# soedinglab/MMseqs2

Measured on AMD Instinct MI355X. Metric: sw_gcells_per_s, higher is better.
Workload: dtype int16

## Files before the change

### mmseqs2_amd/csrc/mmgpu_internal.h

```cpp
#ifndef MMGPU_INTERNAL_H
#define MMGPU_INTERNAL_H

#include <hip/hip_runtime.h>
#include <stdint.h>
#include <cstdlib>
#include <cstring>

#include <algorithm>
#include <array>
#include <string>
#include <map>
#include <mutex>
#include <chrono>
#include <memory>
#include <vector>
#include <thread>
#include <atomic>

#include "../../include/mmgpu.h"
#include "nucl_core.h"
#include "block_plan.h"

namespace mmgpu {

struct DeviceDb {
    uint8_t *res = nullptr;
    uint32_t *off4 = nullptr;
    uint32_t *len = nullptr;
    uint32_t n = 0;
    uint32_t max_len = 0;
    uint64_t total_residues = 0;
    int alphabet = 0;
    size_t res_bytes = 0;
};

struct TargetView {
    const uint8_t *res = nullptr;
    const uint32_t *off4 = nullptr;
    const uint32_t *len = nullptr;
    uint32_t n = 0;
    uint32_t max_len = 0;
    const uint32_t *h_len = nullptr;
};

struct SwMaskGatherArgs {
    const uint8_t *src_res;
    const uint32_t *src_off4, *src_len;
    const uint32_t *src_id;
    uint8_t *dst_res;
    const uint32_t *dst_off4;
    const uint32_t *span_off;
    const mmgpu_sw_span *spans;
    uint32_t span_base;
    uint32_t mask_letter;
    uint32_t n_pairs;
};
hipError_t launch_sw_mask_gather(const SwMaskGatherArgs &A, hipStream_t stream);

struct SwJob {
    uint32_t query;
    uint32_t hit_begin;
    uint32_t hit_end;
    uint32_t shape;
};

struct SwLaunch {
    const SwJob *jobs;
    uint32_t n_jobs;
    const uint8_t *q_res;
    const int8_t *q_cb;
    const uint32_t *q_off;
    const int32_t *q_bias;
    const int32_t *q_minstart;
    const int8_t *q_prof;
    const uint32_t *q_prof_off;
    const uint8_t *t_res;
    const uint32_t *t_off4;
    const uint32_t *t_len;
    const uint32_t *hit_target;
    const uint32_t *hit_out;
    mmgpu_sw_hit *out;
    const int8_t *mat;
    int alphabet;
    int gap_open, gap_extend;
    uint2 *scratch;
    uint32_t scratch_cols;
    uint32_t *scratch_busy;
    uint32_t scratch_slots;
    uint32_t resident_lds = 0;
    const uint32_t *q_hit_count;
    uint32_t hit_stride;
    int rev_mode = 0;
    int rev_only = 0;
    const uint8_t *rev_force = nullptr;
    int half_wide = 1;
};

constexpr int SW_PF_MAX_LIST = 16384;
constexpr int SW_FROM_PF_STAT_SLOTS = 64;

struct SwFromPfArgs {
    const mmgpu_pf_hit *pf_hits;
    uint32_t pf_stride;
    const uint32_t *hit_count;
    uint32_t stride;
    const uint32_t *q_off;
    const uint32_t *t_len;
    uint32_t *hit_target, *hit_out;
    unsigned long long *cells, *pairs;
    uint32_t *count_copy;
    uint32_t *slot_target;
};

constexpr int SW_REV_JOB_MAX = 1024;
hipError_t launch_sw_rev_multi(const SwLaunch &L, size_t lds_bytes, hipStream_t stream);
hipError_t launch_sw_from_pf(const SwFromPfArgs &A, uint32_t nq, hipStream_t stream);
uint32_t sw_multi_resident_blocks(size_t lds_bytes, bool both_passes, int compute_units);

#ifndef MMGPU_SW_MAX_R
#define MMGPU_SW_MAX_R 28
#endif
constexpr int SW_MAX_R = MMGPU_SW_MAX_R;
static_assert(SW_MAX_R >= 16 && SW_MAX_R <= 32, "multi-tile bodies exist for 8..32 rows per lane: a query cut into tiles gets at least SW_MAX_R / 2");
#ifndef MMGPU_SW_MIN_WAVES
#define MMGPU_SW_MIN_WAVES 2
#endif
constexpr int SW_MIN_WAVES = MMGPU_SW_MIN_WAVES;
#ifndef MMGPU_SW_GROUPS
#define MMGPU_SW_GROUPS 4
#endif
constexpr int SW_GROUPS = MMGPU_SW_GROUPS;
static_assert(SW_GROUPS == 3 || SW_GROUPS == 4, "three or four kernel groups");
constexpr int SW_GROUP0_MAX_R = 12;
constexpr int SW_GROUP1_MAX_R = 24;
__host__ __device__ constexpr int sw_group_of(bool multi, int R) {
    return multi ? SW_GROUPS - 1 : (R <= SW_GROUP0_MAX_R ? 0 : (R <= SW_GROUP1_MAX_R ? 1 : 2));
}
int sw_shape_group(uint32_t shape);
hipError_t launch_sw(const SwLaunch &L, int group, size_t lds_bytes, bool both_passes, hipStream_t stream);
#ifndef MMGPU_SW_HALF
#define MMGPU_SW_HALF 1
#endif
bool launch_sw_half(const SwLaunch &L, int group, size_t lds_bytes, bool both_passes, hipStream_t stream);
void warm_sw_half();

constexpr int SW_LDS_HEADER = SW_REV_JOB_MAX * 2 + 64;
__host__ __device__ constexpr int lane_stride_bytes(int R) {
    int slots = (R * 2 + 15) / 16;
    if ((slots & 1) == 0) slots += 1;
    return slots * 16;
}
__host__ __device__ constexpr uint32_t sw_profile_bytes(int R, int alphabet, int lanes = 16) {
    return (uint32_t)(alphabet + 1) * (uint32_t)lanes * (uint32_t)lane_stride_bytes(R);
}
#ifndef MMGPU_SW_RESIDENT_LDS
#define MMGPU_SW_RESIDENT_LDS 65536
#endif
constexpr uint32_t SW_RESIDENT_LDS = MMGPU_SW_RESIDENT_LDS;
static_assert(SW_RESIDENT_LDS <= 65536u, "a workgroup asks for at most 64 KB of dynamic LDS");
__host__ __device__ constexpr uint32_t sw_tiles(uint32_t qlen, int R) { return (qlen + 16u * (uint32_t)R - 1u) / (16u * (uint32_t)R); }
__host__ __device__ constexpr bool sw_multi_resident(uint32_t n_tiles, int R, int alphabet, uint32_t budget) {
    return (unsigned long long)n_tiles * sw_profile_bytes(R, alphabet) + (unsigned long long)SW_LDS_HEADER <= (unsigned long long)budget;
}
static_assert(sw_multi_resident(2, 28, 21, 65536) && sw_multi_resident(3, 24, 21, 65536) && !sw_multi_resident(3, 25, 21, 65536) &&
              !sw_multi_resident(4, 22, 21, 65536) && !sw_multi_resident(2, 8, 21, 0), "residency rule");

constexpr uint32_t SW_SHAPE_MULTI = 32, SW_SHAPE_WIDE = 64;
constexpr int SW_WIDE_MIN_R = (16 * SW_MAX_R + 1 + 31) / 32;
static_assert(sw_profile_bytes(SW_MAX_R, 21, 32) == 2 * sw_profile_bytes(SW_MAX_R, 21) &&
              sw_profile_bytes(SW_MAX_R, 21, 32) + SW_LDS_HEADER <= 65536u, "a wide tile fits a workgroup's 64 KB");
static_assert((lane_stride_bytes(SW_MAX_R) / 16) % 2 == 1 && (lane_stride_bytes(SW_WIDE_MIN_R) / 16) % 2 == 1, "odd number of 16-byte slots");
bool sw_wide_enabled();
bool sw_half_wide();

constexpr int SCAN_CLASSES = 5;
constexpr int SCAN_MULTI = SCAN_CLASSES - 1;
constexpr int SCAN_MAX_R = 32;
constexpr int SCAN_ROUND = 32;
constexpr int SCAN_JOB_TARGETS = 16 * SCAN_ROUND;
__host__ __device__ constexpr int scan_class_rows(int cls) { return cls == 0 ? 8 : cls == 1 ? 16 : cls == 2 ? 24 : 32; }
__host__ __device__ constexpr uint32_t scan_cols(uint32_t len, int R) { return (len + (uint32_t)R - 1u) / (uint32_t)R * (uint32_t)R; }
__host__ __device__ constexpr uint32_t scan_park_row_words(uint32_t longest) { return 2u * ((scan_cols(longest, SCAN_MAX_R) + 1u + 15u) & ~15u); }

constexpr uint64_t SCAN_NO_PROFILE = ~0ull;

struct ScanJob {
    uint32_t query;
    uint32_t begin, end;
    uint32_t pad;
};

struct ScanLaunch {
    const ScanJob *jobs;
    uint32_t n_jobs;
    const uint8_t *q_res;
    const int8_t *q_cb;
    const uint32_t *q_off;
    const int32_t *q_cap;
    const int8_t *q_prof;
    const uint64_t *q_prof_off;
    const uint32_t *q_prof_letters;
    const uint8_t *t_res;
    const uint32_t *t_off4, *t_len;
    const uint32_t *order;
    uint32_t n_targets;
    const int8_t *mat;
    int alphabet;
    uint8_t *scores;
    uint32_t *park;
    const uint64_t *park_off;
};
hipError_t launch_scan(const ScanLaunch &L, int cls, uint32_t grid, hipStream_t stream);

struct ScanSelectArgs {
    const uint8_t *scores;
    const uint32_t *t_len;
    uint32_t n_targets;
    const uint32_t *q_ident;
    const uint32_t *q_win;
    int32_t min_score;
    uint32_t max_hits;
    mmgpu_pf_hit *hits;
    uint32_t stride;
    uint32_t *counts;
};
hipError_t launch_scan_select(const ScanSelectArgs &A, uint32_t nq, hipStream_t stream);
void warm_scan();

constexpr uint64_t GSCAN_PAIR_BUDGET = 1ull << 24;

struct SwDenseLists {
    const uint32_t *begin, *count;
    const uint32_t *order;
    const uint64_t *len_prefix;
    uint32_t *d_hit_target, *d_hit_out;
    mmgpu_sw_hit *d_out;
};

struct GscanPlanArgs {
    const uint32_t *order;
    const uint32_t *q_begin, *q_count;
    const uint32_t *q_slot;
    uint32_t q_first, n_queries;
    uint32_t *hit_target, *hit_out;
};
hipError_t launch_gscan_plan(const GscanPlanArgs &A, hipStream_t stream);

struct GscanIdentArgs {
    const uint8_t *q_res;
    const int8_t *q_cb;
    const uint32_t *q_off;
    const int8_t *q_prof;
    const uint32_t *q_prof_off;
    const uint32_t *q_ident;
    const uint8_t *t_res;
    const uint32_t *t_off4;
    const int8_t *mat;
    int alphabet;
    int32_t *ident_score;
};
hipError_t launch_gscan_identity(const GscanIdentArgs &A, uint32_t nq, hipStream_t stream);

struct GscanSelectArgs {
    const mmgpu_sw_hit *out;
    const uint32_t *order;
    const uint32_t *q_begin, *q_count, *q_slot;
    const uint32_t *q_ident;
    const int32_t *ident_score;
    const int32_t *q_min_ev;
    const uint32_t *t_len;
    const uint32_t *q_win;
    int32_t *scores;
    uint32_t n_targets;
    uint32_t q_first;
    int32_t min_score;
    uint32_t max_hits;
    mmgpu_pf_hit *hits;
    uint32_t stride;
    uint32_t *counts;
};
hipError_t launch_gscan_select(const GscanSelectArgs &A, uint32_t n_queries, hipStream_t stream);
void warm_gscan();

constexpr int RESCORE_GROUP = 16;
constexpr int RESCORE_STEP = 4;
constexpr int RESCORE_THREADS = 256;
constexpr int RESCORE_SLACK = 16;

struct RescoreArgs {
    const uint8_t *q_res;
    const uint32_t *q_off4, *q_len;
    const uint8_t *t_res;
    const uint32_t *t_off4, *t_len;
    const int8_t *mat;
    int alphabet;
    const uint32_t *hit_query;
    const mmgpu_rescore_pair *pairs;
// ... 813 lines not shown
```

### mmseqs2_amd/csrc/sw_body.h

```cpp
#pragma once
#include "mmgpu_internal.h"
#include "pf_device.h"

namespace mmgpu {

namespace {

constexpr int GROUP = 16;
constexpr int WAVES = 4;
constexpr int GROUPS_PER_WAVE = 64 / GROUP;
constexpr int HITS_PER_WAVE = 2 * GROUPS_PER_WAVE;
constexpr unsigned NEG2 = 0x80008000u;

typedef short s16x2 __attribute__((ext_vector_type(2)));
typedef unsigned short u16x2 __attribute__((ext_vector_type(2)));

__device__ __forceinline__ unsigned pk_add_sat(unsigned a, unsigned b) {
    return __builtin_bit_cast(unsigned, __builtin_elementwise_add_sat(__builtin_bit_cast(s16x2, a),
                                                                      __builtin_bit_cast(s16x2, b)));
}
__device__ __forceinline__ unsigned pk_max_s(unsigned a, unsigned b) {
    return __builtin_bit_cast(unsigned, __builtin_elementwise_max(__builtin_bit_cast(s16x2, a),
                                                                  __builtin_bit_cast(s16x2, b)));
}
__device__ __forceinline__ unsigned pk_max_u(unsigned a, unsigned b) {
    return __builtin_bit_cast(unsigned, __builtin_elementwise_max(__builtin_bit_cast(u16x2, a),
                                                                  __builtin_bit_cast(u16x2, b)));
}
__device__ __forceinline__ unsigned pk_sub_sat_u(unsigned a, unsigned b) {
    return __builtin_bit_cast(unsigned, __builtin_elementwise_sub_sat(__builtin_bit_cast(u16x2, a),
                                                                      __builtin_bit_cast(u16x2, b)));
}
__device__ __forceinline__ unsigned bfi(unsigned mask, unsigned a, unsigned b) {
    return (a & mask) | (b & ~mask);
}

constexpr int SW_HALF_LIMIT = 2048 - 256;
constexpr int SW_HALF_MAX_GAP = 2048;
constexpr int SW_HALF_MARK = -1;
typedef _Float16 h16x2 __attribute__((ext_vector_type(2)));
__device__ __forceinline__ h16x2 as_h(unsigned a) { return __builtin_bit_cast(h16x2, a); }
__device__ __forceinline__ unsigned as_u(h16x2 a) { return __builtin_bit_cast(unsigned, a); }
__device__ __forceinline__ unsigned h_add(unsigned a, unsigned b) { return as_u(as_h(a) + as_h(b)); }
__device__ __forceinline__ unsigned h_sub(unsigned a, unsigned b) { return as_u(as_h(a) - as_h(b)); }
__device__ __forceinline__ unsigned h_max(unsigned a, unsigned b) {
    return as_u(__builtin_elementwise_maximum(as_h(a), as_h(b)));
}
__device__ __forceinline__ unsigned h_max3(unsigned a, unsigned b, unsigned c) {
    return as_u(__builtin_elementwise_maximum(__builtin_elementwise_maximum(as_h(a), as_h(b)), as_h(c)));
}
__device__ __forceinline__ unsigned short h_bits(int v) { return __builtin_bit_cast(unsigned short, (_Float16)v); }
__device__ __forceinline__ int h_value(unsigned bits) { return (int)(float)__builtin_bit_cast(_Float16, (unsigned short)bits); }
template <int W>
__device__ __forceinline__ unsigned across_rows(unsigned x, unsigned v) {
    static_assert(W == 16 || W == 32, "groups of one or two DPP rows");
    if constexpr (W == 32) x = __builtin_amdgcn_update_dpp(x, v, 0x138 , 0xA, 0x1, false);
    return x;
}
template <int W = GROUP>
__device__ __forceinline__ unsigned from_lane_above(unsigned head, unsigned v) {
    return across_rows<W>(__builtin_amdgcn_update_dpp(head, v, 0x111 , 0xF, 0xF, false), v);
}
template <int W = GROUP>
__device__ __forceinline__ unsigned from_lane_above_or_zero(unsigned v) {
    return across_rows<W>(__builtin_amdgcn_update_dpp(0u, v, 0x111 , 0xF, 0xF, true), v);
}

#ifndef MMGPU_SW_PREFETCH
#define MMGPU_SW_PREFETCH 1
#endif
#define SW_KEEP_IN_ROW(x) asm volatile("" : "+v"(x))

template <int R, int W = GROUP>
struct Tile {
    static constexpr int ROWS = W * R;
    static constexpr int LANE_STRIDE = lane_stride_bytes(R);
    static constexpr int ROW_STRIDE = W * LANE_STRIDE;
};
static_assert(GROUP == 16, "sw_profile_bytes' default and sw_tiles (mmgpu_internal.h) assume 16-lane groups for all but the wide shapes");

template <int R, bool REV, bool HALF = false, int W = GROUP>
__device__ __forceinline__ void build_profile(unsigned char *lds, const uint8_t *q, const int8_t *cb, int qlen,
                                              int tile_base, const int8_t *mat, int alphabet, const int8_t *prof) {
    using T = Tile<R, W>;
    const int total = (alphabet + 1) * T::ROWS;
    for (int idx = threadIdx.x; idx < total; idx += blockDim.x) {
        const int letter = idx / T::ROWS;
        const int row = idx - letter * T::ROWS;
        const int rg = tile_base + row;
        short v = (short)-32768;
        if (letter < alphabet && rg < qlen) {
            const int qi = REV ? (qlen - 1 - rg) : rg;
            v = prof ? (short)prof[letter * qlen + qi] : (short)((int)mat[letter * alphabet + q[qi]] + (int)cb[qi]);
        }
        const int lane = row / R, r = row - lane * R;
        if constexpr (HALF) v = (short)h_bits(v);
        *reinterpret_cast<short *>(lds + letter * T::ROW_STRIDE + lane * T::LANE_STRIDE + r * 2) = v;
    }
}

__device__ __forceinline__ bool sw_rev_wanted(const SwLaunch &L, uint32_t slot, int min_start) {
    const mmgpu_sw_hit &f = L.out[slot];
    const int s = f.score;
    if (L.rev_mode == 2) return s > 0 && L.rev_force[slot] != 0;
    return s > 0 && s >= min_start && !(L.rev_mode == 1 && f.word != 0);
}

constexpr int SW_REV_JOB_HITS = 1024;
static_assert(SW_REV_JOB_HITS == SW_REV_JOB_MAX, "host and kernel disagree on the reverse job size");
struct SwLds {
    uint16_t live[SW_REV_JOB_HITS];
    uint32_t live_wave[WAVES];
    uint32_t next_chunk;
    uint32_t half_flag;
    uint32_t unused[10];
    __device__ unsigned char *profiles() { return reinterpret_cast<unsigned char *>(this + 1); }
};
constexpr int SW_HALF_FLAG_AT = offsetof(SwLds, half_flag);
static_assert(SW_LDS_HEADER == SW_REV_JOB_HITS * 2 + 64 && sizeof(SwLds) == SW_LDS_HEADER && SW_HALF_FLAG_AT == SW_REV_JOB_HITS * 2 + 20 &&
              offsetof(SwLds, next_chunk) == SW_REV_JOB_HITS * 2 + 16, "the header holds the live hits and the scheduling words");
__device__ __forceinline__ SwLds &sw_lds() {
    extern __shared__ __attribute__((aligned(16))) unsigned char lds_all[];
    return *reinterpret_cast<SwLds *>(lds_all);
}
__device__ __forceinline__ uint32_t sw_half_any_marked() { return sw_lds().half_flag; }

struct SwQuery {
    const uint8_t *q;
    const int8_t *cb;
    int qlen, qbias;
    const int8_t *prof;
};
__device__ __forceinline__ SwQuery sw_query(const SwLaunch &L, uint32_t query) {
    const uint32_t qbeg = L.q_off[query];
    SwQuery Q;
    Q.qlen = (int)(L.q_off[query + 1] - qbeg);
    Q.q = L.q_res + qbeg;
    Q.cb = L.q_cb + qbeg;
    Q.qbias = L.q_bias[query];
    Q.prof = nullptr;
    if (L.q_prof_off) {
        const uint32_t po = L.q_prof_off[query];
        if (po != 0xFFFFFFFFu) Q.prof = L.q_prof + po;
    }
    return Q;
}

struct SwProfiles {
    unsigned char *lds;
    int n_tiles;
    uint32_t tile_bytes;
    bool resident;
    bool dynamic;
};
template <int R, bool MULTI>
__device__ __forceinline__ SwProfiles sw_profiles(const SwLaunch &L, int qlen) {
    SwProfiles P;
    P.lds = sw_lds().profiles();
    P.n_tiles = MULTI ? (int)sw_tiles((uint32_t)qlen, R) : 1;
    P.tile_bytes = sw_profile_bytes(R, L.alphabet);
    P.resident = MULTI && sw_multi_resident((uint32_t)P.n_tiles, R, L.alphabet, L.resident_lds);
    P.dynamic = !MULTI || P.resident;
    return P;
}
enum SwBuildAt { SW_AT_JOB_START, SW_AT_PACKED, SW_AT_TILE };
template <SwBuildAt AT, int R, bool REV, bool HALF, bool PACKED, int W>
__device__ __forceinline__ void sw_build_profiles(const SwLaunch &L, const SwQuery &Q, const SwProfiles &P, int tile = 0) {
    using T = Tile<R, W>;
    if (AT == SW_AT_TILE) {
        if (!P.dynamic) {
            __syncthreads();
            build_profile<R, REV, HALF, W>(P.lds, Q.q, Q.cb, Q.qlen, tile * T::ROWS, L.mat, L.alphabet, Q.prof);
            __syncthreads();
        }
    } else if ((AT == SW_AT_PACKED) == PACKED && P.dynamic) {
        for (int t = 0; t < P.n_tiles; ++t)
            build_profile<R, REV, HALF, W>(P.lds + (uint32_t)t * P.tile_bytes, Q.q, Q.cb, Q.qlen, t * T::ROWS, L.mat, L.alphabet, Q.prof);
        __syncthreads();
    }
}

template <bool REV, bool MARKED>
__device__ __forceinline__ uint32_t sw_pack_live(const SwLaunch &L, const SwJob &job, SwLds &H, uint32_t n_hits) {
    const int lane = threadIdx.x & 63;
    const int wave = __builtin_amdgcn_readfirstlane(threadIdx.x >> 6);
    const int min_start = REV ? L.q_minstart[job.query] : 0;
    uint32_t total = 0;
    for (uint32_t base = 0; base < n_hits; base += WAVES * 64) {
        const uint32_t idx = base + threadIdx.x;
        bool pass = false;
        if (idx < n_hits) {
            const uint32_t slot = L.hit_out[job.hit_begin + idx];
            pass = MARKED ? L.out[slot].score == SW_HALF_MARK : sw_rev_wanted(L, slot, min_start);
        }
        const unsigned long long bal = __ballot(pass);
        if (lane == 0) H.live_wave[wave] = (uint32_t)__popcll(bal);
        __syncthreads();
        uint32_t before = 0, round_total = 0;
#pragma unroll
        for (int w = 0; w < WAVES; ++w) {
            const uint32_t c = H.live_wave[w];
            before += w < wave ? c : 0u;
            round_total += c;
        }
        if (pass) H.live[total + before + (uint32_t)__popcll(bal & ((1ull << lane) - 1ull))] = (uint16_t)idx;
        total += round_total;
        __syncthreads();
    }
    return total;
}

template <int W>
__device__ __forceinline__ uint32_t sw_claim_chunk(SwLds &H, bool dynamic, uint32_t it) {
    constexpr int HITS_PER_WAVE = 2 * 64 / W;
    const int lane = threadIdx.x & 63;
    const int wave = __builtin_amdgcn_readfirstlane(threadIdx.x >> 6);
    uint32_t chunk = it * WAVES + wave;
    if (dynamic) {
        if (lane == 0) chunk = atomicAdd(&H.next_chunk, 1u);
        chunk = __builtin_amdgcn_readfirstlane(chunk);
    }
    return chunk * HITS_PER_WAVE;
}

template <bool REV, bool HALF>
__device__ __forceinline__ void sw_write_result(const SwLaunch &L, const SwQuery &Q, unsigned long long key, uint32_t h, int end, int cols) {
    const bool marked = HALF && (unsigned)(key >> 32) > (unsigned)h_bits(SW_HALF_LIMIT);
    const int score = HALF ? (marked ? SW_HALF_MARK : h_value((unsigned)(key >> 32))) : (int)(key >> 32);
    const int col = 0xFFFF - (int)((key >> 16) & 0xFFFFu);
    const int row = 0xFFFF - (int)(key & 0xFFFFu);
    mmgpu_sw_hit *o = L.out + L.hit_out[h];
    if (!REV) {
        mmgpu_sw_hit res;
        res.score = score;
        res.q_end = score ? row : 0;
        res.t_end = score ? col : -1;
        res.q_start = -1;
        res.t_start = -1;
        res.word = (score + Q.qbias >= 255) ? 1 : 0;
        *o = res;
        if (marked) sw_lds().half_flag = 1;
    } else {
        if (cols > 0) {
            o->t_start = (score == o->score) ? end - col : -2;
            o->q_start = (score == o->score) ? Q.qlen - 1 - row : -2;
        }
    }
}

template <int R, bool MULTI, bool REV, bool PF, bool HALF = false, bool MARKED = false, int W = GROUP>
__device__ __forceinline__ void sw_body(const SwLaunch &L, const SwJob job) {
    static_assert(!(HALF || MARKED) || (!MULTI && !REV && !(HALF && MARKED)), "f16 and its int16 re-run: single-tile forward scans");
    static_assert(W == GROUP || (W == 2 * GROUP && !MULTI), "the boundary row of a multi-tile body rotates inside one DPP row");
    constexpr bool PACKED = REV || MARKED;
    constexpr int HITS_PER_WAVE = 2 * 64 / W;
    using T = Tile<R, W>;
    SwLds &H = sw_lds();
    if (MULTI) __builtin_amdgcn_s_setprio(3);
    const int lane = threadIdx.x & 63;
    const int wave = __builtin_amdgcn_readfirstlane(threadIdx.x >> 6);
    const int g = lane & (W - 1);
    const int grp = lane / W;
    const SwQuery Q = sw_query(L, job.query);
    const SwProfiles prof = sw_profiles<R, MULTI>(L, Q.qlen);
    const unsigned go2 = (HALF ? (unsigned)h_bits(L.gap_open) : (unsigned)L.gap_open) * 0x10001u;
    const unsigned ge2 = (HALF ? (unsigned)h_bits(L.gap_extend) : (unsigned)L.gap_extend) * 0x10001u;
    const unsigned pad_letter = (unsigned)L.alphabet;

    if (threadIdx.x == 0) H.next_chunk = 0;
    if (HALF && threadIdx.x == 0) H.half_flag = 0;
    sw_build_profiles<SW_AT_JOB_START, R, REV, HALF, PACKED, W>(L, Q, prof);
    uint32_t n_hits = job.hit_end - job.hit_begin;
    if (PACKED) {
        n_hits = sw_pack_live<REV, MARKED>(L, job, H, n_hits);
        if (n_hits == 0) return;
    }
    sw_build_profiles<SW_AT_PACKED, R, REV, HALF, PACKED, W>(L, Q, prof);
    const uint32_t n_iter = (n_hits + WAVES * HITS_PER_WAVE - 1) / (WAVES * HITS_PER_WAVE);

    for (uint32_t it = 0; prof.dynamic || it < n_iter; ++it) {
        const uint32_t slot0 = sw_claim_chunk<W>(H, prof.dynamic, it);
        if (prof.dynamic && slot0 >= n_hits) break;

        const uint32_t sA = slot0 + grp * 2, sB = sA + 1;
        const bool vA = sA < n_hits, vB = sB < n_hits;
        const uint32_t hA = job.hit_begin + (PACKED ? (uint32_t)H.live[vA ? sA : 0] : sA);
        const uint32_t hB = job.hit_begin + (PACKED ? (uint32_t)H.live[vB ? sB : 0] : sB);
        const uint32_t tA = vA ? L.hit_target[hA] : 0u, tB = vB ? L.hit_target[hB] : 0u;
        const uint8_t *pA = L.t_res + (size_t)L.t_off4[tA] * 4;
        const uint8_t *pB = L.t_res + (size_t)L.t_off4[tB] * 4;
        int colsA = vA ? (int)L.t_len[tA] : 0, colsB = vB ? (int)L.t_len[tB] : 0;
        int r0A = 0, r0B = 0;
        int endA = 0, endB = 0;
        unsigned rev_target = 0xFFFFFFFFu;
        if (REV) {
            mmgpu_sw_hit fa, fb;
            fa.score = 0; fa.q_end = 0; fa.t_end = 0;
            fb = fa;
            if (vA) fa = L.out[L.hit_out[hA]];
            if (vB) fb = L.out[L.hit_out[hB]];
            colsA = vA ? fa.t_end + 1 : 0;
            colsB = vB ? fb.t_end + 1 : 0;
            endA = colsA > 0 ? fa.t_end : 0;
            endB = colsB > 0 ? fb.t_end : 0;
            r0A = colsA > 0 ? Q.qlen - 1 - fa.q_end : 0;
            r0B = colsB > 0 ? Q.qlen - 1 - fb.q_end : 0;
            rev_target = (colsA > 0 ? (unsigned)fa.score & 0xFFFFu : 0xFFFFu) | ((colsB > 0 ? (unsigned)fb.score & 0xFFFFu : 0xFFFFu) << 16);
        }
        int ncols = colsA > colsB ? colsA : colsB;
        ncols = max(ncols, __shfl_xor(ncols, 16));
        ncols = max(ncols, __shfl_xor(ncols, 32));
        ncols = __builtin_amdgcn_readfirstlane(ncols);
        const int nsteps = ncols + W - 1;
        int mincols = colsA < colsB ? colsA : colsB;
        mincols = min(mincols, __shfl_xor(mincols, 16));
        mincols = min(mincols, __shfl_xor(mincols, 32));
        mincols = __builtin_amdgcn_readfirstlane(mincols);

        unsigned long long bestA = 0, bestB = 0;

        uint2 *scr = nullptr;
        unsigned scr_grp = 0;
        if (MULTI) {
            scr = L.scratch + (size_t)((job.shape >> 8) * WAVES + wave) * GROUPS_PER_WAVE * 2 * L.scratch_cols;
            scr_grp = (unsigned)grp * 2u * L.scratch_cols;
        }

        for (int tile = 0; tile < prof.n_tiles; ++tile) {
            const int tile_base = tile * T::ROWS;
            sw_build_profiles<SW_AT_TILE, R, REV, HALF, PACKED, W>(L, Q, prof, tile);
            const unsigned char *const lds_tile = MULTI && prof.resident ? prof.lds + (uint32_t)tile * prof.tile_bytes : prof.lds;
            const uint2 *scr_in = MULTI ? scr + (size_t)((tile + 1) & 1) * L.scratch_cols : nullptr;
            uint2 *scr_out = MULTI ? scr + (size_t)(tile & 1) * L.scratch_cols : nullptr;
            const bool has_above = MULTI && tile > 0;
            const bool has_below = MULTI && tile + 1 < prof.n_tiles;

            unsigned Hp[R], E[R], aux[R];
#pragma unroll
            for (int r = 0; r < R; ++r) { Hp[r] = 0; E[r] = 0; aux[r] = 0; }
            if (REV) {
#pragma unroll
                for (int r = 0; r < R; ++r) {
                    const int rg = tile_base + g * R + r;
                    aux[r] = (rg >= r0A ? 0xFFFFu : 0u) | (rg >= r0B ? 0xFFFF0000u : 0u);
                }
            }
            unsigned vmax = 0, bestcol = 0xFFFFFFFFu;
            unsigned rev_rowA = 0, rev_rowB = 0;
            unsigned Hup_prev = 0;
            unsigned out_H = 0, out_F = 0;

            auto letters4 = [&](const uint8_t *p, int end, int k) -> unsigned {
                if (!REV) return reinterpret_cast<const unsigned *>(p)[k];
                int o = end - 3 - 4 * k;
                o = o < -3 ? -3 : o;
                unsigned w;
                __builtin_memcpy(&w, p + o, 4);
                return w;
            };
            unsigned wA = letters4(pA, endA, 0), wB = letters4(pB, endB, 0);
            unsigned wA_next = letters4(pA, endA, 1), wB_next = letters4(pB, endB, 1);
            uint2 bnd = make_uint2(0, 0), bnd_next = make_uint2(0, 0);
            auto boundary16 = [&](int m) -> uint2 {
                const int last = ncols - 1 < 0 ? 0 : ncols - 1;
                return scr_in[scr_grp + (unsigned)min(16 * m + g - (m > 0 ? 1 : 0), last)];
            };
            if (has_above) {
                bnd = boundary16(0);
                bnd_next = boundary16(1);
            }

            constexpr int ND = (R + 1) / 2;
            unsigned pav_next[PF ? ND : 1], pbv_next[PF ? ND : 1];
            auto load_rows = [&](unsigned letters, unsigned *pav, unsigned *pbv) {
                const unsigned a = letters & 0xFFu, b = (letters >> 8) & 0xFFu;
                const uint4 *rowA = reinterpret_cast<const uint4 *>(lds_tile + a * T::ROW_STRIDE + g * T::LANE_STRIDE);
                const uint4 *rowB = reinterpret_cast<const uint4 *>(lds_tile + b * T::ROW_STRIDE + g * T::LANE_STRIDE);
#pragma unroll
                for (int k = 0; k < ND / 4; ++k) {
                    const uint4 pa = rowA[k], pb = rowB[k];
                    pav[4 * k] = pa.x; pav[4 * k + 1] = pa.y; pav[4 * k + 2] = pa.z; pav[4 * k + 3] = pa.w;
                    pbv[4 * k] = pb.x; pbv[4 * k + 1] = pb.y; pbv[4 * k + 2] = pb.z; pbv[4 * k + 3] = pb.w;
                }
                if constexpr (ND % 4 >= 2) {
                    const uint2 pa = *reinterpret_cast<const uint2 *>(rowA + ND / 4);
                    const uint2 pb = *reinterpret_cast<const uint2 *>(rowB + ND / 4);
                    pav[(ND / 4) * 4] = pa.x; pav[(ND / 4) * 4 + 1] = pa.y;
                    pbv[(ND / 4) * 4] = pb.x; pbv[(ND / 4) * 4 + 1] = pb.y;
                }
                if constexpr (ND % 2 == 1) {
                    pav[ND - 1] = reinterpret_cast<const unsigned *>(rowA)[ND - 1];
                    pbv[ND - 1] = reinterpret_cast<const unsigned *>(rowB)[ND - 1];
                }
            };
            unsigned let = pad_letter * 0x101u;
            constexpr bool LETTER_BLOCKS = MULTI || REV || R >= 7;
            constexpr bool LETTER_QUEUE = !MULTI && R < 7;
            unsigned long long lq = 0;
            auto letter_block = [&](int k) {
                if (!LETTER_BLOCKS) return;
                unsigned a = wA, b = wB;
                if (4 * k + 4 > mincols) {
                    const unsigned pad4 = pad_letter * 0x01010101u;
                    const int na = min(max(colsA - 4 * k, 0), 4), nb = min(max(colsB - 4 * k, 0), 4);
                    const unsigned ma = REV ? ~(unsigned)(0xFFFFFFFFull >> (8 * na)) : (unsigned)((1ull << (8 * na)) - 1ull);
                    const unsigned mb = REV ? ~(unsigned)(0xFFFFFFFFull >> (8 * nb)) : (unsigned)((1ull << (8 * nb)) - 1ull);
                    a = bfi(ma, a, pad4);
                    b = bfi(mb, b, pad4);
                }
                const unsigned lo = __builtin_amdgcn_perm(b, a, REV ? 0x06020703u : 0x05010400u);
                const unsigned hi = __builtin_amdgcn_perm(b, a, REV ? 0x04000501u : 0x07030602u);
                lq = ((unsigned long long)hi << 32) | lo;
            };
            auto head_letters = [&](int c, int j) -> unsigned {
                if (LETTER_BLOCKS && LETTER_QUEUE) { const unsigned v = (unsigned)lq; lq >>= 16; return v; }
                if (LETTER_BLOCKS) return (unsigned)(lq >> (16 * j));
                const unsigned sh = (unsigned)(REV ? 3 - j : j) * 8u;
                const unsigned la0 = __builtin_amdgcn_ubfe(wA, sh, 8u);
                const unsigned lb0 = __builtin_amdgcn_ubfe(wB, sh, 8u);
                return (c < colsA ? la0 : pad_letter) | ((c < colsB ? lb0 : pad_letter) << 8);
            };
            letter_block(0);
            let = from_lane_above<W>(head_letters(0, 0), let);
            if (PF) load_rows(let, pav_next, pbv_next);

            for (int s0 = -1; s0 < nsteps; s0 += 4) {
            if (MULTI && s0 > 0 && ((s0 + 1) & 15) == 0) {
                bnd = bnd_next;
                if (has_above) bnd_next = boundary16(((s0 + 1) >> 4) + 1);
            }
            const int jn = min(4, nsteps - s0);
#pragma nounroll
            for (int j = s0 < 0 ? 1 : 0; j < jn; ++j) {
                const int s = s0 + j;
                if (has_below && s >= GROUP) {
                    if (g == GROUP - 1) (scr_out + (s - GROUP))[scr_grp] = make_uint2(out_H, out_F);
                }
                const unsigned Hup = MULTI ? from_lane_above<W>(bnd.x, out_H) : from_lane_above_or_zero<W>(out_H);
                unsigned f = MULTI ? from_lane_above<W>(bnd.y, out_F) : from_lane_above_or_zero<W>(out_F);
                if (MULTI) {
                    bnd.x = __builtin_amdgcn_update_dpp(bnd.x, bnd.x, 0x12F, 0xF, 0xF, false);
                    bnd.y = __builtin_amdgcn_update_dpp(bnd.y, bnd.y, 0x12F, 0xF, 0xF, false);
                }
                unsigned pav[ND], pbv[ND];
                if (PF) {
#pragma unroll
                    for (int k = 0; k < ND; ++k) { pav[k] = pav_next[k]; pbv[k] = pbv_next[k]; }
                } else {
                    load_rows(let, pav, pbv);
                }

                unsigned hd = Hup_prev;
                Hup_prev = Hup;
                unsigned cmax = 0;
                unsigned pre[R], es[R];
#pragma unroll
                for (int r = 0; r < R; ++r) {
                    unsigned P = __builtin_amdgcn_perm(pbv[r / 2], pav[r / 2], (r & 1) ? 0x07060302u : 0x05040100u);
                    if (REV) P = __builtin_amdgcn_bitop3_b32(aux[r], P, NEG2, 0xCA);
                    if constexpr (HALF) {
                        pre[r] = h_add(r == 0 ? hd : Hp[r - 1], P);
                        es[r] = h_sub(E[r], ge2);
                    } else {
                        pre[r] = pk_max_s(pk_add_sat(r == 0 ? hd : Hp[r - 1], P), E[r]);
                        es[r] = pk_sub_sat_u(E[r], ge2);
                    }
                }
                let = from_lane_above<W>(head_letters(s + 1, j), let);
                if (PF) load_rows(let, pav_next, pbv_next);
#pragma unroll
                for (int r = 0; r < R; ++r) {
                    unsigned h;
                    if constexpr (HALF) {
                        h = h_max3(pre[r], E[r], f);
                        const unsigned fs = h_sub(f, ge2);
                        const unsigned t = h_sub(h, go2);
                        cmax = r == 0 ? h : h_max(cmax, h);
                        f = h_max3(fs, t, 0u);
                        E[r] = h_max3(es[r], t, 0u);
                    } else {
                        h = pk_max_s(pre[r], f);
                        const unsigned fs = pk_sub_sat_u(f, ge2);
                        const unsigned t = pk_sub_sat_u(h, go2);
                        cmax = pk_max_u(cmax, h);
                        f = pk_max_u(fs, t);
                        E[r] = pk_max_u(es[r], t);
                    }
                    SW_KEEP_IN_ROW(E[r]);
                    Hp[r] = h;
                }
                out_H = Hp[R - 1];
                out_F = f;

                const int col = s - g;

                const unsigned nm = pk_max_u(vmax, cmax);
                if (nm != vmax) {
                    const unsigned diff = nm ^ vmax;
                    if (!REV) {
                        const unsigned mask = ((diff & 0xFFFFu) ? 0xFFFFu : 0u) | ((diff >> 16) ? 0xFFFF0000u : 0u);
                        bestcol = bfi(mask, ((unsigned)col & 0xFFFFu) * 0x10001u, bestcol);
#pragma unroll
                        for (int r = 0; r < R; ++r) aux[r] = bfi(mask, Hp[r], aux[r]);
                    } else {
                        const unsigned x = nm ^ rev_target;
                        const bool hitA = (diff & 0xFFFFu) && !(x & 0xFFFFu), hitB = (diff >> 16) && !(x >> 16);
                        if (hitA | hitB) {
                            asm volatile("" ::: "memory");
                            unsigned ra = 0, rb = 0;
#pragma unroll
                            for (int r = R - 1; r >= 0; --r) {
                                if ((Hp[r] & 0xFFFFu) == (rev_target & 0xFFFFu)) ra = (unsigned)r;
                                if ((Hp[r] >> 16) == (rev_target >> 16)) rb = (unsigned)r;
                            }
                            if (hitA) { bestcol = (bestcol & 0xFFFF0000u) | ((unsigned)col & 0xFFFFu); rev_rowA = ra; }
                            if (hitB) { bestcol = (bestcol & 0xFFFFu) | ((unsigned)col << 16); rev_rowB = rb; }
                        }
                    }
                    vmax = nm;
                }
            }
            {
                wA = wA_next; wB = wB_next;
                const int k = ((s0 + 1) >> 2) + 2;
                wA_next = letters4(pA, endA, k); wB_next = letters4(pB, endB, k);
                letter_block(k - 1);
            }
            }
            if (has_below && ncols > 0 && g == GROUP - 1) (scr_out + (ncols - 1))[scr_grp] = make_uint2(out_H, out_F);

            unsigned rowA_first = rev_rowA, rowB_first = rev_rowB;
            unsigned sA = vmax & 0xFFFFu, sB = vmax >> 16;
            if (!REV) {
#pragma unroll
                for (int r = R - 1; r >= 0; --r) {
                    if ((aux[r] & 0xFFFFu) == sA) rowA_first = (unsigned)r;
                    if ((aux[r] >> 16) == sB) rowB_first = (unsigned)r;
                }
            } else {
                sA = sA == (rev_target & 0xFFFFu) ? sA : 0u;
                sB = sB == (rev_target >> 16) ? sB : 0u;
            }
            const unsigned rgA = (unsigned)(tile_base + g * R) + rowA_first;
            const unsigned rgB = (unsigned)(tile_base + g * R) + rowB_first;
            unsigned long long keyA = sA ? ((unsigned long long)sA << 32) | ((0xFFFFu - (bestcol & 0xFFFFu)) << 16) | (0xFFFFu - rgA) : 0ull;
            unsigned long long keyB = sB ? ((unsigned long long)sB << 32) | ((0xFFFFu - (bestcol >> 16)) << 16) | (0xFFFFu - rgB) : 0ull;
#pragma unroll
            for (int m = 1; m < W; m <<= 1) {
                const unsigned long long oa = __shfl_xor(keyA, m), ob = __shfl_xor(keyB, m);
                keyA = oa > keyA ? oa : keyA;
                keyB = ob > keyB ? ob : keyB;
            }
            bestA = keyA > bestA ? keyA : bestA;
            bestB = keyB > bestB ? keyB : bestB;
        }

        if (g == 0) {
            if (vA) sw_write_result<REV, HALF>(L, Q, bestA, hA, endA, colsA);
            if (vB) sw_write_result<REV, HALF>(L, Q, bestB, hB, endB, colsB);
        }
    }
}

template <int R, bool MULTI, bool BOTH>
constexpr bool SW_PREFETCHES = MMGPU_SW_PREFETCH && !MULTI && (BOTH || sw_group_of(false, R) < 2);
template <int R, bool MULTI, bool BOTH, int W = GROUP>
__device__ __forceinline__ void sw_passes(const SwLaunch &L, const SwJob &job) {
    constexpr bool PF = SW_PREFETCHES<R, MULTI, BOTH>;
    if (!(BOTH && L.rev_only)) sw_body<R, MULTI, false, PF, false, false, W>(L, job);
    if constexpr (BOTH && !MULTI) {
        __threadfence_block();
        __syncthreads();
        sw_body<R, MULTI, true, PF, false, false, W>(L, job);
    }
}

#ifndef MMGPU_SW_WAVES_G0F
#define MMGPU_SW_WAVES_G0F 4
#endif
#ifndef MMGPU_SW_WAVES_G0B
#define MMGPU_SW_WAVES_G0B 2
#endif
#ifndef MMGPU_SW_WAVES_G1F
#define MMGPU_SW_WAVES_G1F 3
#endif
#ifndef MMGPU_SW_WAVES_G1B
#define MMGPU_SW_WAVES_G1B 2
#endif
constexpr int sw_waves_floor(int G, bool BOTH) {
    return G == 0 ? (BOTH ? MMGPU_SW_WAVES_G0B : MMGPU_SW_WAVES_G0F) : (G == 1 ? (BOTH ? MMGPU_SW_WAVES_G1B : MMGPU_SW_WAVES_G1F) : SW_MIN_WAVES);
}
constexpr int sw_waves_cap(int G, bool BOTH) { return G == 1 && BOTH ? MMGPU_SW_WAVES_G1B : 8; }

__device__ __forceinline__ bool sw_clip_job(const SwLaunch &L, SwJob &job) {
    if (L.q_hit_count) {
        const uint32_t lim = job.query * L.hit_stride + L.q_hit_count[job.query];
        job.hit_end = job.hit_end < lim ? job.hit_end : lim;
        if (job.hit_end <= job.hit_begin) return false;
    }
    return true;
}

__device__ __forceinline__ void sw_claim_scratch(const SwLaunch &L, SwJob &job) {
    __shared__ uint32_t scratch_slot;
    if (threadIdx.x == 0) {
        uint32_t s = blockIdx.x % L.scratch_slots;
        while (atomicCAS(&L.scratch_busy[s], 0u, 1u) != 0u) s = s + 1 == L.scratch_slots ? 0u : s + 1;
        scratch_slot = s;
    }
    __syncthreads();
    job.shape = (job.shape & 0xFFu) | (scratch_slot << 8);
}
__device__ __forceinline__ void sw_release_scratch(const SwLaunch &L, const SwJob &job) {
    __syncthreads();
    if (threadIdx.x == 0) {
        __threadfence();
        atomicExch(&L.scratch_busy[job.shape >> 8], 0u);
    }
}

enum SwKind { SW_SINGLE, SW_MULTI, SW_WIDE };
constexpr bool sw_shape_exists(SwKind kind, int R) {
    return R <= SW_MAX_R && (kind != SW_MULTI || R >= 8) && (kind != SW_WIDE || R >= SW_WIDE_MIN_R);
}
#define MMGPU_SW_EACH_R(X)                                                                                                          \
    X(1) X(2) X(3) X(4) X(5) X(6) X(7) X(8) X(9) X(10) X(11) X(12) X(13) X(14) X(15) X(16) X(17) X(18) X(19) X(20) X(21) X(22) X(23) \
    X(24) X(25) X(26) X(27) X(28) X(29) X(30) X(31) X(32)
template <int G, typename F>
__device__ __forceinline__ void sw_dispatch_shape(uint32_t shape, F f) {
    static_assert(GROUP == 16 && SW_SHAPE_MULTI == 32 && SW_SHAPE_WIDE == 64, "the shape codes of the dispatch: 16-lane groups, + 32 multi-tile, + 64 wide");
#define MMGPU_SW_CASE(R, KIND, BASE)                                                                                                \
    case BASE + (R) - 1:                                                                                                            \
        if constexpr (sw_shape_exists(KIND, R) && sw_group_of(KIND == SW_MULTI, R) == G)                                            \
            f(std::integral_constant<int, R>(), std::integral_constant<SwKind, KIND>());                                            \
        break;
#define MMGPU_SW_CASES(R) MMGPU_SW_CASE(R, SW_SINGLE, 0) MMGPU_SW_CASE(R, SW_MULTI, SW_SHAPE_MULTI) MMGPU_SW_CASE(R, SW_WIDE, SW_SHAPE_WIDE)
    switch (shape & 0xFFu) {
        MMGPU_SW_EACH_R(MMGPU_SW_CASES)
        default: break;
    }
#undef MMGPU_SW_CASES
#undef MMGPU_SW_CASE
}

}

}
```

### mmseqs2_amd/csrc/sw_kernel.hip

```cpp
#include "mmgpu_internal.h"
#include "pf_device.h"
#include "sw_body.h"

namespace mmgpu {

namespace {

template <int G, bool BOTH>
__global__ __launch_bounds__(WAVES * 64)
__attribute__((amdgpu_waves_per_eu(sw_waves_floor(G, BOTH), sw_waves_cap(G, BOTH)))) void sw_kernel(SwLaunch L) {
    SwJob job = L.jobs[blockIdx.x];
    if (!sw_clip_job(L, job)) return;
    const bool claims = G == SW_GROUPS - 1 && (job.shape & 0xFFu) >= SW_SHAPE_MULTI && (job.shape & 0xFFu) < SW_SHAPE_WIDE;
    if (claims) sw_claim_scratch(L, job);
    sw_dispatch_shape<G>(job.shape, [&](auto r, auto kind) __attribute__((always_inline)) {
        sw_passes<decltype(r)::value, decltype(kind)::value == SW_MULTI, BOTH, decltype(kind)::value == SW_WIDE ? 2 * GROUP : GROUP>(L, job);
    });
    if (claims) sw_release_scratch(L, job);
}

__global__ __launch_bounds__(WAVES * 64) __attribute__((amdgpu_waves_per_eu(SW_MIN_WAVES))) void sw_rev_multi_kernel(SwLaunch L) {
    SwJob job = L.jobs[blockIdx.x];
    if (!sw_clip_job(L, job)) return;
    sw_claim_scratch(L, job);
    sw_dispatch_shape<SW_GROUPS - 1>(job.shape, [&](auto r, auto kind) __attribute__((always_inline)) {
        if constexpr (decltype(kind)::value == SW_MULTI) sw_body<decltype(r)::value, true, true, false>(L, job);
    });
    sw_release_scratch(L, job);
}

__global__ __launch_bounds__(256) void sw_from_pf_kernel(SwFromPfArgs A) {
    extern __shared__ uint32_t key[];
    const uint32_t q = blockIdx.x;
    unsigned long long *const stat = A.cells + (size_t)(blockIdx.x % (uint32_t)SW_FROM_PF_STAT_SLOTS) * 3;
    const uint32_t n = min(A.hit_count[q], A.stride);
    const mmgpu_pf_hit *hits = A.pf_hits + (size_t)q * A.pf_stride;
    uint32_t np2 = 1;
    while (np2 < n) np2 <<= 1;
    unsigned long long cells = 0;
    const uint32_t qlen = A.q_off[q + 1] - A.q_off[q];
    for (uint32_t k = threadIdx.x; k < np2; k += 256) {
        uint32_t v = 0xFFFFFFFFu;
        if (k < n) {
            const uint32_t len = A.t_len[hits[k].id];
            v = ((0xFFFFu - min(len, 0xFFFFu)) << 16) | k;
            cells += (unsigned long long)qlen * len;
        }
        key[k] = v;
    }
    __syncthreads();
    const uint32_t base = q * A.stride;
    if (n <= 512) {
        for (uint32_t i = threadIdx.x; i < n; i += 256) {
            const uint32_t mine = key[i];
            uint32_t r = 0;
            for (uint32_t j = 0; j < n; j++) r += key[j] < mine ? 1u : 0u;
            A.hit_target[base + r] = hits[i].id;
            A.hit_out[base + r] = base + i;
            A.slot_target[base + i] = hits[i].id;
            if (r == 0) atomicMax(stat + 2, (unsigned long long)(0xFFFFu - (mine >> 16)));
        }
    } else {
    block_bitonic_sort<256>(np2, [&](uint32_t i, uint32_t j) { return key[i] > key[j]; }, [&](uint32_t i, uint32_t j) { exchange_at(key, i, j); });
    for (uint32_t r = threadIdx.x; r < n; r += 256) {
        const uint32_t k = key[r] & 0xFFFFu;
        A.hit_target[base + r] = hits[k].id;
        A.hit_out[base + r] = base + k;
        A.slot_target[base + r] = hits[r].id;
    }
    if (threadIdx.x == 0 && n) atomicMax(stat + 2, (unsigned long long)(0xFFFFu - (key[0] >> 16)));
    }
    for (uint32_t r = n + threadIdx.x; r < A.stride; r += 256) {
        A.hit_target[base + r] = 0;
        A.hit_out[base + r] = base + r;
        A.slot_target[base + r] = 0;
    }
    if (threadIdx.x == 0) A.count_copy[q] = n;
    wave_sum_to(stat, cells);
    if (threadIdx.x == 0 && n) atomicAdd(stat + 1, (unsigned long long)n);
}

}

hipError_t launch_sw_from_pf(const SwFromPfArgs &A, uint32_t nq, hipStream_t stream) {
    static_assert((SW_PF_MAX_LIST & (SW_PF_MAX_LIST - 1)) == 0 && (size_t)SW_PF_MAX_LIST * sizeof(uint32_t) <= 65536,
                  "SW_PF_MAX_LIST: a power of two whose dwords fit 64 KB of dynamic LDS");
    if (A.stride > (uint32_t)SW_PF_MAX_LIST) return hipErrorInvalidValue;
    if (nq == 0) return hipSuccess;
    uint32_t np2 = 1;
    while (np2 < A.stride) np2 <<= 1;
    const size_t lds = (size_t)np2 * sizeof(uint32_t);
    if (lds > 65536) return hipErrorInvalidValue;
    const hipError_t attr = hipFuncSetAttribute(reinterpret_cast<const void *>(sw_from_pf_kernel),
                                                hipFuncAttributeMaxDynamicSharedMemorySize, 65536);
    if (attr != hipSuccess) return attr;
    hipLaunchKernelGGL(sw_from_pf_kernel, dim3(nq), dim3(256), lds, stream, A);
    return hipGetLastError();
}

uint32_t sw_multi_resident_blocks(size_t lds_bytes, bool both_passes, int compute_units) {
    int per_cu = 0;
    const size_t lds = lds_bytes + SW_LDS_HEADER;
    hipError_t e = both_passes ? hipOccupancyMaxActiveBlocksPerMultiprocessor(&per_cu, sw_kernel<SW_GROUPS - 1, true>, WAVES * 64, lds)
                               : hipOccupancyMaxActiveBlocksPerMultiprocessor(&per_cu, sw_kernel<SW_GROUPS - 1, false>, WAVES * 64, lds);
    if (e == hipSuccess && both_passes) {
        int rev = 0;
        if (hipOccupancyMaxActiveBlocksPerMultiprocessor(&rev, sw_rev_multi_kernel, WAVES * 64, lds) == hipSuccess) per_cu = std::max(per_cu, rev);
    }
    if (e != hipSuccess || per_cu < 1) per_cu = 8;
    per_cu = per_cu + 1 > 8 ? 8 : per_cu + 1;
    return (uint32_t)per_cu * (uint32_t)(compute_units > 0 ? compute_units : 256);
}

hipError_t launch_sw_rev_multi(const SwLaunch &L, size_t lds_bytes, hipStream_t stream) {
    if (L.n_jobs == 0) return hipSuccess;
    hipLaunchKernelGGL(sw_rev_multi_kernel, dim3(L.n_jobs), dim3(WAVES * 64), lds_bytes + SW_LDS_HEADER, stream, L);
    return hipGetLastError();
}

int sw_shape_group(uint32_t shape) {
    const uint32_t kind = shape >= SW_SHAPE_WIDE ? SW_SHAPE_WIDE : (shape >= SW_SHAPE_MULTI ? SW_SHAPE_MULTI : 0u);
    return sw_group_of(kind == SW_SHAPE_MULTI, (int)(shape - kind) + 1);
}

static bool env_switch(const char *name, bool unset) {
    const char *v = getenv(name);
    return v && *v ? atoi(v) != 0 : unset;
}
bool sw_wide_enabled() {
    static const bool on = env_switch("MMGPU_SW_WIDE", true);
    return on;
}
bool sw_half_wide() {
    static const bool on = env_switch("MMGPU_SW_HALF_WIDE", true);
    return on;
}

static bool sw_half_eligible(const SwLaunch &L) {
    return MMGPU_SW_HALF && !L.rev_only && L.gap_open >= 0 && L.gap_open <= SW_HALF_MAX_GAP && L.gap_extend >= 0 &&
           L.gap_extend <= SW_HALF_MAX_GAP;
}

hipError_t launch_sw(const SwLaunch &L, int group, size_t lds_bytes, bool both_passes, hipStream_t stream) {
    if (L.n_jobs == 0) return hipSuccess;
    if (sw_half_eligible(L) && launch_sw_half(L, group, lds_bytes, both_passes, stream)) return hipGetLastError();
    dim3 grid(L.n_jobs), block(WAVES * 64);
    const size_t lds = lds_bytes + SW_LDS_HEADER;
    switch (group * 2 + (both_passes ? 1 : 0)) {
        case 0: hipLaunchKernelGGL((sw_kernel<0, false>), grid, block, lds, stream, L); break;
        case 1: hipLaunchKernelGGL((sw_kernel<0, true>), grid, block, lds, stream, L); break;
        case 2: hipLaunchKernelGGL((sw_kernel<1, false>), grid, block, lds, stream, L); break;
        case 3: hipLaunchKernelGGL((sw_kernel<1, true>), grid, block, lds, stream, L); break;
        case 4: hipLaunchKernelGGL((sw_kernel<2, false>), grid, block, lds, stream, L); break;
        case 5: hipLaunchKernelGGL((sw_kernel<2, true>), grid, block, lds, stream, L); break;
        case 6: hipLaunchKernelGGL((sw_kernel<SW_GROUPS - 1, false>), grid, block, lds, stream, L); break;
        case 7: hipLaunchKernelGGL((sw_kernel<SW_GROUPS - 1, true>), grid, block, lds, stream, L); break;
        default: return hipErrorInvalidValue;
    }
    return hipGetLastError();
}

void warm_sw() {
    hipFuncAttributes a;
    (void)hipFuncGetAttributes(&a, reinterpret_cast<const void *>(&sw_rev_multi_kernel));
    if (MMGPU_SW_HALF) warm_sw_half();
}

}
```

Baseline: 5016.

## Run reverse Smith-Waterman pass in packed f16 reusing forward profile mirrored

Adds a new kernel that runs both the forward and the reverse (start-finding) passes in packed half precision for single-tile shapes. The reverse pass reuses the forward query profile by reading lane slices and rows mirrored, with a padding offset, so it never rebuilds a reversed profile. Hits whose scores overflow the f16 range fall back to int16 forward and reverse re-runs. The aim is to take the reverse pass off the slower int16 path and skip its profile builds, at the cost of more code paths and extra complexity in the precision fallback.

```diff
diff --git a/mmseqs2_amd/csrc/mmgpu_internal.h b/mmseqs2_amd/csrc/mmgpu_internal.h
--- a/mmseqs2_amd/csrc/mmgpu_internal.h
+++ b/mmseqs2_amd/csrc/mmgpu_internal.h
@@ -143,6 +143,8 @@
 #endif
 bool launch_sw_half(const SwLaunch &L, int group, size_t lds_bytes, bool both_passes, hipStream_t stream);
 void warm_sw_half();
+bool launch_sw_hrev(const SwLaunch &L, int group, size_t lds_bytes, bool both_passes, hipStream_t stream);
+void warm_sw_hrev();
 
 constexpr int SW_LDS_HEADER = SW_REV_JOB_MAX * 2 + 64;
 __host__ __device__ constexpr int lane_stride_bytes(int R) {
diff --git a/mmseqs2_amd/csrc/sw_body.h b/mmseqs2_amd/csrc/sw_body.h
--- a/mmseqs2_amd/csrc/sw_body.h
+++ b/mmseqs2_amd/csrc/sw_body.h
@@ -36,6 +36,7 @@
 }
 
 constexpr int SW_HALF_LIMIT = 2048 - 256;
+constexpr unsigned NEGH2 = 0xF800F800u;
 constexpr int SW_HALF_MAX_GAP = 2048;
 constexpr int SW_HALF_MARK = -1;
 typedef _Float16 h16x2 __attribute__((ext_vector_type(2)));
@@ -191,7 +192,8 @@
         bool pass = false;
         if (idx < n_hits) {
             const uint32_t slot = L.hit_out[job.hit_begin + idx];
-            pass = MARKED ? L.out[slot].score == SW_HALF_MARK : sw_rev_wanted(L, slot, min_start);
+            if constexpr (REV && MARKED) pass = sw_rev_wanted(L, slot, min_start) && L.out[slot].score > SW_HALF_LIMIT;
+            else pass = MARKED ? L.out[slot].score == SW_HALF_MARK : sw_rev_wanted(L, slot, min_start);
         }
         const unsigned long long bal = __ballot(pass);
         if (lane == 0) H.live_wave[wave] = (uint32_t)__popcll(bal);
@@ -250,7 +252,8 @@
 
 template <int R, bool MULTI, bool REV, bool PF, bool HALF = false, bool MARKED = false, int W = GROUP>
 __device__ __forceinline__ void sw_body(const SwLaunch &L, const SwJob job) {
-    static_assert(!(HALF || MARKED) || (!MULTI && !REV && !(HALF && MARKED)), "f16 and its int16 re-run: single-tile forward scans");
+    static_assert(!(HALF || MARKED) || (!MULTI && !(HALF && MARKED)), "f16 and its int16 re-run: single-tile scans");
+    constexpr bool HREV = HALF && REV;
     static_assert(W == GROUP || (W == 2 * GROUP && !MULTI), "the boundary row of a multi-tile body rotates inside one DPP row");
     constexpr bool PACKED = REV || MARKED;
     constexpr int HITS_PER_WAVE = 2 * 64 / W;
@@ -268,14 +271,15 @@
     const unsigned pad_letter = (unsigned)L.alphabet;
 
     if (threadIdx.x == 0) H.next_chunk = 0;
-    if (HALF && threadIdx.x == 0) H.half_flag = 0;
-    sw_build_profiles<SW_AT_JOB_START, R, REV, HALF, PACKED, W>(L, Q, prof);
+    if (HALF && !REV && threadIdx.x == 0) H.half_flag = 0;
+    if constexpr (!HREV) sw_build_profiles<SW_AT_JOB_START, R, REV, HALF, PACKED, W>(L, Q, prof);
     uint32_t n_hits = job.hit_end - job.hit_begin;
     if (PACKED) {
         n_hits = sw_pack_live<REV, MARKED>(L, job, H, n_hits);
         if (n_hits == 0) return;
     }
-    sw_build_profiles<SW_AT_PACKED, R, REV, HALF, PACKED, W>(L, Q, prof);
+    if constexpr (!HREV) sw_build_profiles<SW_AT_PACKED, R, REV, HALF, PACKED, W>(L, Q, prof);
+    const int pad = HREV ? T::ROWS - Q.qlen : 0;
     const uint32_t n_iter = (n_hits + WAVES * HITS_PER_WAVE - 1) / (WAVES * HITS_PER_WAVE);
 
     for (uint32_t it = 0; prof.dynamic || it < n_iter; ++it) {
@@ -303,9 +307,11 @@
             colsB = vB ? fb.t_end + 1 : 0;
             endA = colsA > 0 ? fa.t_end : 0;
             endB = colsB > 0 ? fb.t_end : 0;
-            r0A = colsA > 0 ? Q.qlen - 1 - fa.q_end : 0;
-            r0B = colsB > 0 ? Q.qlen - 1 - fb.q_end : 0;
-            rev_target = (colsA > 0 ? (unsigned)fa.score & 0xFFFFu : 0xFFFFu) | ((colsB > 0 ? (unsigned)fb.score & 0xFFFFu : 0xFFFFu) << 16);
+            r0A = colsA > 0 ? Q.qlen - 1 - fa.q_end + pad : 0;
+            r0B = colsB > 0 ? Q.qlen - 1 - fb.q_end + pad : 0;
+            const unsigned ta = HALF ? (unsigned)h_bits(fa.score) : (unsigned)fa.score & 0xFFFFu;
+            const unsigned tb = HALF ? (unsigned)h_bits(fb.score) : (unsigned)fb.score & 0xFFFFu;
+            rev_target = (colsA > 0 ? ta : 0xFFFFu) | ((colsB > 0 ? tb : 0xFFFFu) << 16);
         }
         int ncols = colsA > colsB ? colsA : colsB;
         ncols = max(ncols, __shfl_xor(ncols, 16));
@@ -328,7 +334,7 @@
 
         for (int tile = 0; tile < prof.n_tiles; ++tile) {
             const int tile_base = tile * T::ROWS;
-            sw_build_profiles<SW_AT_TILE, R, REV, HALF, PACKED, W>(L, Q, prof, tile);
+            if constexpr (!HREV) sw_build_profiles<SW_AT_TILE, R, REV, HALF, PACKED, W>(L, Q, prof, tile);
             const unsigned char *const lds_tile = MULTI && prof.resident ? prof.lds + (uint32_t)tile * prof.tile_bytes : prof.lds;
             const uint2 *scr_in = MULTI ? scr + (size_t)((tile + 1) & 1) * L.scratch_cols : nullptr;
             uint2 *scr_out = MULTI ? scr + (size_t)(tile & 1) * L.scratch_cols : nullptr;
@@ -374,8 +380,9 @@
             unsigned pav_next[PF ? ND : 1], pbv_next[PF ? ND : 1];
             auto load_rows = [&](unsigned letters, unsigned *pav, unsigned *pbv) {
                 const unsigned a = letters & 0xFFu, b = (letters >> 8) & 0xFFu;
-                const uint4 *rowA = reinterpret_cast<const uint4 *>(lds_tile + a * T::ROW_STRIDE + g * T::LANE_STRIDE);
-                const uint4 *rowB = reinterpret_cast<const uint4 *>(lds_tile + b * T::ROW_STRIDE + g * T::LANE_STRIDE);
+                const int slice = HREV ? W - 1 - g : g;
+                const uint4 *rowA = reinterpret_cast<const uint4 *>(lds_tile + a * T::ROW_STRIDE + slice * T::LANE_STRIDE);
+                const uint4 *rowB = reinterpret_cast<const uint4 *>(lds_tile + b * T::ROW_STRIDE + slice * T::LANE_STRIDE);
 #pragma unroll
                 for (int k = 0; k < ND / 4; ++k) {
                     const uint4 pa = rowA[k], pb = rowB[k];
@@ -456,8 +463,9 @@
                 unsigned pre[R], es[R];
 #pragma unroll
                 for (int r = 0; r < R; ++r) {
-                    unsigned P = __builtin_amdgcn_perm(pbv[r / 2], pav[r / 2], (r & 1) ? 0x07060302u : 0x05040100u);
-                    if (REV) P = __builtin_amdgcn_bitop3_b32(aux[r], P, NEG2, 0xCA);
+                    const int pr = HREV ? R - 1 - r : r;
+                    unsigned P = __builtin_amdgcn_perm(pbv[pr / 2], pav[pr / 2], (pr & 1) ? 0x07060302u : 0x05040100u);
+                    if (REV) P = __builtin_amdgcn_bitop3_b32(aux[r], P, HALF ? NEGH2 : NEG2, 0xCA);
                     if constexpr (HALF) {
                         pre[r] = h_add(r == 0 ? hd : Hp[r - 1], P);
                         es[r] = h_sub(E[r], ge2);
@@ -541,8 +549,8 @@
                 sA = sA == (rev_target & 0xFFFFu) ? sA : 0u;
                 sB = sB == (rev_target >> 16) ? sB : 0u;
             }
-            const unsigned rgA = (unsigned)(tile_base + g * R) + rowA_first;
-            const unsigned rgB = (unsigned)(tile_base + g * R) + rowB_first;
+            const unsigned rgA = (unsigned)(tile_base + g * R - pad) + rowA_first;
+            const unsigned rgB = (unsigned)(tile_base + g * R - pad) + rowB_first;
             unsigned long long keyA = sA ? ((unsigned long long)sA << 32) | ((0xFFFFu - (bestcol & 0xFFFFu)) << 16) | (0xFFFFu - rgA) : 0ull;
             unsigned long long keyB = sB ? ((unsigned long long)sB << 32) | ((0xFFFFu - (bestcol >> 16)) << 16) | (0xFFFFu - rgB) : 0ull;
 #pragma unroll
diff --git a/mmseqs2_amd/csrc/sw_hrev_kernel.hip b/mmseqs2_amd/csrc/sw_hrev_kernel.hip
--- /dev/null
+++ b/mmseqs2_amd/csrc/sw_hrev_kernel.hip
@@ -0,0 +1,59 @@
+#include "mmgpu_internal.h"
+#include "pf_device.h"
+#include "sw_body.h"
+
+namespace mmgpu {
+
+namespace {
+
+template <int R, int W>
+constexpr bool SW_HREV_PREFETCHES = !(W == GROUP && R == 12);
+static_assert(sw_group_of(false, 12) == 0 && sw_group_of(false, 13) == 1, "R = 12 is the largest body of group 0");
+template <int R, int W = GROUP>
+__device__ __forceinline__ void sw_hrev_passes(const SwLaunch &L, const SwJob &job) {
+    constexpr bool PF = SW_PREFETCHES<R, false, true>;
+    sw_body<R, false, false, PF, true, false, W>(L, job);
+    __threadfence_block();
+    __syncthreads();
+    sw_body<R, false, true, PF && SW_HREV_PREFETCHES<R, W>, true, false, W>(L, job);
+    if (sw_half_any_marked()) {
+        __syncthreads();
+        sw_body<R, false, false, PF, false, true, W>(L, job);
+        __threadfence_block();
+        __syncthreads();
+        sw_body<R, false, true, PF, false, true, W>(L, job);
+    }
+}
+
+template <int G>
+__global__ __launch_bounds__(WAVES * 64)
+__attribute__((amdgpu_waves_per_eu(sw_waves_floor(G, true), sw_waves_cap(G, true)))) void sw_hrev_kernel(SwLaunch L) {
+    SwJob job = L.jobs[blockIdx.x];
+    if (!sw_clip_job(L, job)) return;
+    sw_dispatch_shape<G>(job.shape, [&](auto r, auto kind) __attribute__((always_inline)) {
+        if constexpr (decltype(kind)::value != SW_MULTI)
+            sw_hrev_passes<decltype(r)::value, decltype(kind)::value == SW_WIDE ? 2 * GROUP : GROUP>(L, job);
+    });
+}
+
+}
+
+bool launch_sw_hrev(const SwLaunch &L, int group, size_t lds_bytes, bool both_passes, hipStream_t stream) {
+    if (group < 0 || group > 2 || (group == 2 && SW_GROUPS != 4)) return false;
+    if (!both_passes || L.rev_mode == 2 || !L.half_wide) return false;
+    dim3 grid(L.n_jobs), block(WAVES * 64);
+    const size_t lds = lds_bytes + SW_LDS_HEADER;
+    switch (group) {
+        case 0: hipLaunchKernelGGL((sw_hrev_kernel<0>), grid, block, lds, stream, L); break;
+        case 1: hipLaunchKernelGGL((sw_hrev_kernel<1>), grid, block, lds, stream, L); break;
+        default: hipLaunchKernelGGL((sw_hrev_kernel<2>), grid, block, lds, stream, L); break;
+    }
+    return true;
+}
+
+void warm_sw_hrev() {
+    hipFuncAttributes a;
+    (void)hipFuncGetAttributes(&a, reinterpret_cast<const void *>(&sw_hrev_kernel<0>));
+}
+
+}
diff --git a/mmseqs2_amd/csrc/sw_kernel.hip b/mmseqs2_amd/csrc/sw_kernel.hip
--- a/mmseqs2_amd/csrc/sw_kernel.hip
+++ b/mmseqs2_amd/csrc/sw_kernel.hip
@@ -131,6 +131,10 @@
     static const bool on = env_switch("MMGPU_SW_WIDE", true);
     return on;
 }
+static bool sw_half_rev() {
+    static const bool on = env_switch("MMGPU_SW_HALF_REV", true);
+    return on;
+}
 bool sw_half_wide() {
     static const bool on = env_switch("MMGPU_SW_HALF_WIDE", true);
     return on;
@@ -143,6 +147,7 @@
 
 hipError_t launch_sw(const SwLaunch &L, int group, size_t lds_bytes, bool both_passes, hipStream_t stream) {
     if (L.n_jobs == 0) return hipSuccess;
+    if (sw_half_eligible(L) && sw_half_rev() && launch_sw_hrev(L, group, lds_bytes, both_passes, stream)) return hipGetLastError();
     if (sw_half_eligible(L) && launch_sw_half(L, group, lds_bytes, both_passes, stream)) return hipGetLastError();
     dim3 grid(L.n_jobs), block(WAVES * 64);
     const size_t lds = lds_bytes + SW_LDS_HEADER;
@@ -164,6 +169,7 @@
     hipFuncAttributes a;
     (void)hipFuncGetAttributes(&a, reinterpret_cast<const void *>(&sw_rev_multi_kernel));
     if (MMGPU_SW_HALF) warm_sw_half();
+    if (MMGPU_SW_HALF) warm_sw_hrev();
 }
 
 }
```

Measured after the change: 5014. No clear change (-0.0%).
